# broadinstitute/gatk-bwamem-jni

Hardware: AMD Instinct MI355X
Metric: 150bp reads aligned/sec vs GRCh38-scale reference (1/2/4/8 MI355X) (higher is better)
Workload: dtype u8/int32/int64; 1 GPU; 10000000 x 150bp single-end synthetic reads per GPU vs synthetic GRCh38-scale genome (3100000000 bp, 24 contigs, 5% diverged repeats), full index in HBM; reads_per_gpu=10000000, read_len=150, genome_bp=3100000000, genome=iid, response_bytes=542940344, parallelism=read-sharded x1, no collectives, hip_hw_queues=4, paired_end=False

## Files before the change

gatk-bwamem-jni_amd/csrc/bwamem_types.h:

```cpp
#pragma once
#include <stdint.h>
#include <stddef.h>
#include <hip/hip_runtime.h>

struct MemOpt {
    int a, b;
    int o_del, e_del;
    int o_ins, e_ins;
    int pen_unpaired;
    int pen_clip5, pen_clip3;
    int w;
    int zdrop;
    uint64_t max_mem_intv;
    int T;
    int flag;
    int min_seed_len;
    int min_chain_weight;
    int max_chain_extend;
    float split_factor;
    int split_width;
    int max_occ;
    int max_chain_gap;
    int n_threads;
    int chunk_size;
    float mask_level;
    float drop_ratio;
    float XA_drop_ratio;
    float mask_level_redun;
    float mapQ_coef_len;
    int mapQ_coef_fac;
    int max_ins;
    int max_matesw;
    int max_XA_hits, max_XA_hits_alt;
    int8_t mat[25];
};
static_assert(sizeof(MemOpt) == 168, "mem_opt_t ABI (BwaMemAligner.java:137)");

struct MemPestat { int low, high; int failed; double avg, std; };
static_assert(sizeof(MemPestat) == 32, "mem_pestat_t ABI");

struct PairTab { const double* t; int64_t lo[4]; int32_t n[4], off[4]; };

enum {
    MEM_F_PE = 0x2, MEM_F_NOPAIRING = 0x4, MEM_F_ALL = 0x8, MEM_F_NO_MULTI = 0x10,
    MEM_F_NO_RESCUE = 0x20, MEM_F_PRIMARY5 = 0x800
};

struct DevIndex {
    const uint4* occ;
    const uint32_t* sa_lo;
    const uint8_t*  sa_hi;
    const uint8_t*  pac;
    const int64_t*  ann_offset;
    const int32_t*  ann_len;
    const int32_t*  ann_is_alt;
    const int32_t*  ann_name_off;
    const char*     names;
    const double*   log_tab;
    uint64_t primary, L2[5], seq_len;
    int64_t  l_pac;
    int32_t  n_seqs, sa_intv, log_tab_n, sa_shift;
    int32_t  n_cu, lds_bytes;
};

struct Intv { uint64_t x0, x1, size, info; };

struct Seed { int64_t rbeg; int32_t qbeg, len, score, next; };

struct Chain {
    int64_t pos;
    int32_t n, first, rid;
    uint32_t w;
    int32_t kept, is_alt;
    int32_t seed0;
    int32_t last;
    float frac_rep;
    int32_t pad_;
};

struct AlnReg {
    int64_t rb, re;
    int32_t qb, qe;
    int32_t rid;
    int32_t score, truesc, sub, alt_sc, csub, sub_n, w, seedcov, secondary, secondary_all, seedlen0;
    int32_t n_comp, is_alt;
    float frac_rep;
    int32_t pad_;
    uint64_t hash;
};

struct SwJob { int64_t rb; int32_t read, tag, l_ms, is_rev, tlen, xtra, q_off, pad_; };
struct KswR { int score, te, qe, score2, te2, tb, qb; };

struct DevCounters {
    unsigned long long n_ext, n_lf, n_sa, n_dp_cells, n_ref_bases, n_reads;
    unsigned long long dbg[10];
};

enum { ERR_INTV_CAP = 1, ERR_OUT_CAP = 2, ERR_CIGAR_CAP = 4, ERR_LONG_READ = 8, ERR_SCRATCH = 16, ERR_BTREE = 32, ERR_BAD_REG = 64, ERR_JOB_CAP = 128, ERR_ZPOOL = 256, ERR_RESCUE_CAP = 512 };

#define BT_NODE_INTS 40

struct TileView {
    int32_t n_reads;
    int32_t max_len;
    int64_t read_id0;
    const int64_t* seq_off;
    uint8_t* seq;
    int32_t intv_cap;
    Intv* intv;
    int32_t* n_intv;
    Intv* smem_scratch;
    int32_t smem_cap;
    int32_t* l_rep;
    int32_t* n_seeds;
// ... 32 lines not shown
```

gatk-bwamem-jni_amd/csrc/k_seed.hip:

```cpp
#include "dev_common.h"
#include "wave_ops.h"
#include "kernels.h"

DEV uint32_t mask16(int n)
{
    n = n < 0 ? 0 : n > 16 ? 16 : n;
    return (uint32_t)(0x5555555500000000ull >> (n << 1));
}
DEV void cnt_word_m(uint32_t x, uint32_t m, uint32_t& c1, uint32_t& c2, uint32_t& c3)
{
    const uint32_t lo = x & m, hi = (x >> 1) & m;
    c3 += __popc(hi & lo);
    c2 += __popc(hi & ~lo);
    c1 += __popc(~hi & lo);
}
DEV void extend_sm(const DevIndex& ix, uint64_t x0, uint64_t x1, uint64_t size, int c, bool is_back, uint64_t& o0, uint64_t& o1, uint64_t& osz)
{
    const uint64_t xa = is_back ? x0 : x1, xb = is_back ? x1 : x0;
    const uint64_t k = xa - 1, l = xa - 1 + size;
    const uint64_t kk = k - (k >= ix.primary), ll = l - (l >= ix.primary);
    const uint64_t bk = kk >> 6, bl = ll >> 6;
    const uint4* pk = ix.occ + 2 * bk;
    const uint4* pl = ix.occ + 2 * bl;
    const uint4 ck = pk[0], sk = pk[1], cl = pl[0], sl = pl[1];
    const int nk = (int)(kk & 63) + 1, nl = (int)(ll & 63) + 1;
    uint32_t a1 = 0, a2 = 0, a3 = 0, b1 = 0, b2 = 0, b3 = 0;
    cnt_word_m(sk.x, mask16(nk), a1, a2, a3);       cnt_word_m(sl.x, mask16(nl), b1, b2, b3);
    cnt_word_m(sk.y, mask16(nk - 16), a1, a2, a3);  cnt_word_m(sl.y, mask16(nl - 16), b1, b2, b3);
    cnt_word_m(sk.z, mask16(nk - 32), a1, a2, a3);  cnt_word_m(sl.z, mask16(nl - 32), b1, b2, b3);
    cnt_word_m(sk.w, mask16(nk - 48), a1, a2, a3);  cnt_word_m(sl.w, mask16(nl - 48), b1, b2, b3);
    const uint64_t tk1 = ((uint64_t)(ck.w & 0xffu) << 32 | ck.x) + a1, tk2 = ((uint64_t)(ck.w >> 8 & 0xffu) << 32 | ck.y) + a2, tk3 = ((uint64_t)(ck.w >> 16 & 0xffu) << 32 | ck.z) + a3;
    const uint64_t tl1 = ((uint64_t)(cl.w & 0xffu) << 32 | cl.x) + b1, tl2 = ((uint64_t)(cl.w >> 8 & 0xffu) << 32 | cl.y) + b2, tl3 = ((uint64_t)(cl.w >> 16 & 0xffu) << 32 | cl.z) + b3;
    const uint64_t s1 = tl1 - tk1, s2 = tl2 - tk2, s3 = tl3 - tk3;
    const uint64_t s0 = (ll - kk) - s1 - s2 - s3;
    const uint64_t tk0 = kk + 1 - tk1 - tk2 - tk3;
    const uint64_t tkc = c == 0 ? tk0 : c == 1 ? tk1 : c == 2 ? tk2 : tk3;
    const uint64_t sc = c == 0 ? s0 : c == 1 ? s1 : c == 2 ? s2 : s3;
    const uint64_t l2c = c == 0 ? ix.L2[0] : c == 1 ? ix.L2[1] : c == 2 ? ix.L2[2] : ix.L2[3];
    uint64_t other = xb + (xa <= ix.primary && xa + size - 1 >= ix.primary);
    other += (c < 3 ? s3 : 0) + (c < 2 ? s2 : 0) + (c < 1 ? s1 : 0);
    const uint64_t na = l2c + 1 + tkc;
    o0 = is_back ? na : other;
    o1 = is_back ? other : na;
    osz = sc;
}

struct CandStack {
    uint32_t *v0, *v1, *v2;
    uint16_t* v2n;
    uint4* spill;
    int K, spill_cap;
    bool narrow;
    static __device__ uint32_t pack2(uint64_t x0, uint64_t size, int end) { return (uint32_t)(x0 >> 32) | (uint32_t)(size >> 32) << 5 | (uint32_t)end << 10; }
    __device__ uint32_t hi_get(int e) const {
        const int s = (e & (K - 1)) * 64;
        if (!narrow) return v2[s];
        const uint32_t h = v2n[s];
        return (h & 7u) | (h >> 3 & 7u) << 5 | (h >> 6) << 10;
    }
    __device__ void hi_put(int e, uint32_t w2) {
        const int s = (e & (K - 1)) * 64;
        if (!narrow) v2[s] = w2;
        else v2n[s] = (uint16_t)((w2 & 7u) | (w2 >> 5 & 7u) << 3 | (w2 >> 10) << 6);
    }
    __device__ bool push(int e, uint64_t x0, uint64_t size, int end) {
        const int s = (e & (K - 1)) * 64;
        if (e >= K) {
            if (e - K >= spill_cap) return false;
            uint4 t; t.x = v0[s]; t.y = v1[s]; t.z = hi_get(e); t.w = 0;
            spill[(size_t)(e - K) * 64] = t;
        }
        v0[s] = (uint32_t)x0; v1[s] = (uint32_t)size; hi_put(e, pack2(x0, size, end));
        return true;
    }
    __device__ void put(int e, int n, uint64_t x0, uint64_t size, int end) {
        if (e >= n - K) { const int s = (e & (K - 1)) * 64; v0[s] = (uint32_t)x0; v1[s] = (uint32_t)size; hi_put(e, pack2(x0, size, end)); }
        else { uint4 t; t.x = (uint32_t)x0; t.y = (uint32_t)size; t.z = pack2(x0, size, end); t.w = 0; spill[(size_t)e * 64] = t; }
    }
    __device__ void get(int e, int n, uint64_t& x0, uint64_t& size, int& end) const {
        uint32_t a, b, w2;
        if (e >= n - K) { const int s = (e & (K - 1)) * 64; a = v0[s]; b = v1[s]; w2 = hi_get(e); }
        else { const uint4 t = spill[(size_t)e * 64]; a = t.x; b = t.y; w2 = t.z; }
        x0 = (uint64_t)(w2 & 31) << 32 | a; size = (uint64_t)(w2 >> 5 & 31) << 32 | b; end = (int)(w2 >> 10);
    }
};

__global__ void k_encode(uint8_t* seq, int64_t n_bytes)
{
    int64_t i = (int64_t)blockIdx.x * blockDim.x + threadIdx.x;
    int64_t stride = (int64_t)gridDim.x * blockDim.x;
    for (; i < n_bytes; i += stride) {
        uint8_t c = seq[i];
        if (c >= 4) {
            uint8_t u = c & 0xdf;
            c = u == 'A' ? 0 : u == 'C' ? 1 : u == 'G' ? 2 : u == 'T' ? 3 : 4;
            seq[i] = c;
        }
    }
}

enum { S_IDLE = 0, S_NEXT = 1, S_FWD = 2, S_BWD = 3, S_P3 = 4 };
#define SEED_EL_CAP 4

template <bool LDSQ>
__global__ void __launch_bounds__(64) k_seed(DevIndex ix, MemOpt opt, TileView tv, int K, int refill_min, int narrow)
{
    HIP_DYNAMIC_SHARED(uint32_t, lds)
    const int lane = threadIdx.x;
    CandStack V;
    V.narrow = narrow != 0;
    V.v0 = lds + lane; V.v1 = V.v0 + K * 64; V.v2 = V.v1 + K * 64; V.K = K;
    V.v2n = (uint16_t*)(lds + 2 * K * 64) + lane;
    V.spill = (uint4*)tv.smem_scratch + (size_t)blockIdx.x * tv.smem_cap * 64 + lane; V.spill_cap = tv.smem_cap;
    uint32_t* el = lds + (narrow ? 5 * K * 32 : 3 * K * 64) + lane;
    uint32_t* sq = el + SEED_EL_CAP * 64;
    unsigned int* work = (unsigned int*)(tv.err + 8);
    const int min_seed_len = opt.min_seed_len;
    const int split_len = (int)(opt.min_seed_len * opt.split_factor + .499);
    const uint64_t max_intv3 = (uint64_t)(int64_t)(int)opt.max_mem_intv;

    int st = S_IDLE, r = 0, len = 0, pass = 1, x = 0, sx = 0, i = 0, k2 = 0, old_n = 0, mem_n = 0;
    int nf = 0, lo = 0, rd = 0, wr = 0, c = -1, ret = 0, end = 0, n_el = 0;
    uint64_t min_intv = 1, last_start = 0, last_sz = 0, ik0 = 0, ik1 = 0, iks = 0;
    bool any = false, ovf = false, exhausted = false, el_ok = true;
    const uint8_t* qg = tv.seq;
    Intv* mem = tv.intv;
    uint32_t n_ext = 0;

    uint64_t qwin = 0;
    const uint8_t* qwin_at = nullptr;
    auto qat_g = [&](int p) -> int {
        const uint8_t* a = qg + p;
        const uint8_t* al = a - ((uintptr_t)a & 7);
        if (al != qwin_at) { qwin_at = al; qwin = *(const uint64_t*)al; }
        return (int)(qwin >> (((uintptr_t)a & 7) << 3) & 0xffu);
    };
#define QAT(p) (LDSQ ? (int)(sq[((p) >> 3) * 64] >> (((p) & 7) << 2) & 15u) : qat_g(p))
#define FINISH() do { fin = true; st = S_IDLE; } while (0)
#define MEM_PUSH(X0, SZ, INFO) do { if (mem_n >= tv.intv_cap) ovf = true; else { Intv v_; v_.x0 = (X0); v_.x1 = 0; v_.size = (SZ); v_.info = (INFO); mem[mem_n++] = v_; } } while (0)
#define PUSH_IK() do { if (V.push(nf, ik0, iks, end)) ++nf; else ovf = true; } while (0)
#define BEGIN_BWD() do { ret = end; lo = 0; rd = wr = nf - 1; i = sx - 1; c = i >= 0 ? QAT(i) : 4; c = c < 4 ? c : -1; st = S_BWD; } while (0)

    for (;;) {
        bool fin = false;
        const unsigned long long idle = __ballot(st == S_IDLE);
        if (idle != 0ull && !exhausted && (__popcll(idle) >= refill_min || idle == ~0ull)) {
            const int n_need = __popcll(idle);
            unsigned int base = 0;
            if (lane == 0) base = atomicAdd(work, (unsigned int)n_need);
            base = (unsigned int)__shfl((int)base, 0);
            if (base + (unsigned int)n_need >= (unsigned int)tv.n_reads) exhausted = true;
            bool fresh = false;
            if (st == S_IDLE) {
                const unsigned int cand = base + (unsigned int)__popcll(idle & ((1ull << lane) - 1ull));
                if (cand < (unsigned int)tv.n_reads) {
                    r = (int)cand; fresh = true;
                    const int64_t off = tv.seq_off[r];
                    len = (int)(tv.seq_off[r + 1] - off - 1);
                    qg = tv.seq + off;
                    mem = tv.intv + (size_t)r * tv.intv_cap;
                    mem_n = 0; ovf = false; pass = 1; x = 0; st = S_NEXT; n_el = 0; el_ok = true;
                }
            }
            if (LDSQ) {
                unsigned long long got = __ballot(fresh);
                while (got) {
                    const int l = __ffsll((long long)got) - 1;
                    got &= got - 1ull;
                    const int rr = __shfl(r, l);
                    const int64_t off = tv.seq_off[rr];
                    const int nb = (int)(tv.seq_off[rr + 1] - off) - 1;
                    for (int k = lane; k * 8 < nb; k += 64) {
                        uint32_t wd = 0;
                        uint32_t by[8];
#pragma unroll
                        for (int b = 0; b < 8; ++b) { const int pos = k * 8 + b; by[b] = tv.seq[off + (pos < nb ? pos : nb)]; }
#pragma unroll
                        for (int b = 0; b < 8; ++b) wd |= (k * 8 + b < nb ? by[b] & 15u : 4u) << (b << 2);
                        sq[k * 64 + (l - lane)] = wd;
                    }
                }
                __syncthreads();
            }
            if (fresh && len < min_seed_len) { tv.n_intv[r] = 0; st = S_IDLE; }
        }
        if (__ballot(st != S_IDLE) == 0ull) break;

        if (st == S_NEXT) {
            int nx = -1;
            bool p3 = false;
            uint64_t nmin = 1;
            if (pass == 1) {
                if (x >= len) { pass = 2; old_n = mem_n; k2 = 0; }
                else if (QAT(x) > 3) ++x;
                else nx = x;
            } else if (pass == 2 && el_ok) {
                if (k2 >= n_el) { pass = 3; x = 0; if (!(opt.max_mem_intv > 0)) FINISH(); }
                else {
                    const uint32_t wd = el[k2 * 64];
                    const int m = (int)(wd & 0x1ffffu);
                    if (QAT(m) > 3) ++k2;
                    else { nx = m; nmin = (uint64_t)(wd >> 17) + 1; }
                }
            } else if (pass == 2) {
                if (k2 >= old_n) { pass = 3; x = 0; if (!(opt.max_mem_intv > 0)) FINISH(); }
                else {
                    const uint64_t psz = mem[k2].size, pinfo = mem[k2].info;
                    const int s0 = (int)(pinfo >> 32), e0 = (int)(int32_t)pinfo;
                    if (e0 - s0 < split_len || psz > (uint64_t)(int64_t)opt.split_width) ++k2;
                    else {
                        const int m = (s0 + e0) >> 1;
                        if (QAT(m) > 3) ++k2;
                        else { nx = m; nmin = psz + 1; }
                    }
                }
            } else {
                if (x >= len) FINISH();
                else if (QAT(x) > 3) ++x;
                else { nx = x; p3 = true; }
            }
            if (nx >= 0) {
                const int b = QAT(nx);
                const uint64_t lb = b == 0 ? ix.L2[0] : b == 1 ? ix.L2[1] : b == 2 ? ix.L2[2] : ix.L2[3];
                const uint64_t lb1 = b == 0 ? ix.L2[1] : b == 1 ? ix.L2[2] : b == 2 ? ix.L2[3] : ix.L2[4];
                const uint64_t lc = b == 0 ? ix.L2[3] : b == 1 ? ix.L2[2] : b == 2 ? ix.L2[1] : ix.L2[0];
                ik0 = lb + 1; iks = lb1 - lb; ik1 = lc + 1;
                sx = nx; i = sx + 1;
                if (p3) st = S_P3;
                else { min_intv = nmin; end = sx + 1; nf = 0; any = false; st = S_FWD; }
            }
        }

        bool need = false, bw = false, back = false;
        int rc = 0, pend = 0;
        uint64_t r0 = 0, r1 = 0, rs = 0;
        bool fwd_end = false;
        if (st == S_FWD || st == S_P3) {
            const int cq = i < len ? QAT(i) : 4;
            if (cq < 4) { need = true; rc = 3 - cq; r0 = ik0; r1 = ik1; rs = iks; }
            else if (st == S_FWD) fwd_end = true;
            else { x = i < len ? i + 1 : len; st = S_NEXT; }
        }
        if (st == S_BWD) {
            V.get(rd, nf, r0, rs, pend);
            bw = true;
            if (c >= 0) { need = true; back = true; rc = c; }
        }

        uint64_t o0 = 0, o1 = 0, os = 0, em0 = 0, ems = 0, emi = 0;
        bool emit = false;
        if (need) { extend_sm(ix, r0, r1, rs, rc, back, o0, o1, os); ++n_ext; }

        if (bw) {
            if (!need || os < min_intv) {
                if (wr == nf - 1 && (!any || (uint64_t)(i + 1) < last_start)) {
                    any = true; last_start = (uint64_t)(i + 1);
                    if (pend - (i + 1) >= min_seed_len) {
                        emit = true; em0 = r0; ems = rs; emi = (uint64_t)(i + 1) << 32 | (uint32_t)pend;
                        if (pass == 1 && pend - (i + 1) >= split_len && rs <= (uint64_t)(int64_t)opt.split_width) {
                            if (n_el < SEED_EL_CAP && rs < 32768u) el[n_el * 64] = (uint32_t)((i + 1 + pend) >> 1) | (uint32_t)rs << 17;
                            else el_ok = false;
                            ++n_el;
                        }
                    }
                }
            } else if (wr == nf - 1 || os != last_sz) {
                V.put(wr, nf, o0, os, pend); --wr; last_sz = os;
            }
            --rd;
            if (rd < lo) {
                if (wr == nf - 1) { if (pass == 1) x = ret; else ++k2; st = S_NEXT; }
                else { lo = wr + 1; rd = wr = nf - 1; --i; c = i >= 0 ? QAT(i) : 4; c = c < 4 ? c : -1; }
            }
        } else if (st == S_FWD && (need || fwd_end)) {
            const bool push = fwd_end || os != iks;
            const bool stop = fwd_end || (push && os < min_intv);
            if (push) PUSH_IK();
            if (stop) BEGIN_BWD();
            else { ik0 = o0; ik1 = o1; iks = os; end = i + 1; ++i; }
        } else if (need) {
            if (os < max_intv3 && i - sx >= min_seed_len) {
                if (os > 0) { emit = true; em0 = o0; ems = os; emi = (uint64_t)sx << 32 | (uint32_t)(i + 1); }
                x = i + 1; st = S_NEXT;
            } else { ik0 = o0; ik1 = o1; iks = os; ++i; }
        }
        if (emit) MEM_PUSH(em0, ems, emi);
        if (ovf) FINISH();
        if (fin) {
            tv.n_intv[r] = ovf ? 0 : mem_n;
            if (ovf) atomicOr(tv.err, ERR_INTV_CAP);
        }
    }
#undef QAT
#undef FINISH
#undef MEM_PUSH
#undef PUSH_IK
#undef BEGIN_BWD
    unsigned long long tot = n_ext;
    for (int o = 32; o > 0; o >>= 1) tot += __shfl_down(tot, o);
    if (lane == 0) { count_add(&tv.cnt->n_ext, tot); }
}

__global__ void k_seed_fin(MemOpt opt, TileView tv)
{
    const int r = blockIdx.x * blockDim.x + threadIdx.x;
    if (r >= tv.n_reads) return;
    Intv* a = tv.intv + (size_t)r * tv.intv_cap;
    const int n = tv.n_intv[r];
    for (int i = 1; i < n; ++i) {
        Intv t = a[i];
        int j = i;
        while (j > 0 && a[j - 1].info > t.info) { a[j] = a[j - 1]; --j; }
        a[j] = t;
    }
    int n_seeds = 0, l_rep = 0, b = 0, e = 0;
    int32_t* iso = tv.intv_seed_off + (size_t)r * tv.intv_cap;
    for (int i = 0; i < n; ++i) {
        const Intv p = a[i];
        const int sb = (int)(p.info >> 32), se = (int)(uint32_t)p.info;
        iso[i] = n_seeds;
        {
            int64_t step = p.size > (uint64_t)(int64_t)opt.max_occ ? (int64_t)(p.size / (uint64_t)opt.max_occ) : 1;
            int64_t c = ((int64_t)p.size + step - 1) / step;
            n_seeds += (int)(c < opt.max_occ ? c : opt.max_occ);
        }
        if (p.size <= (uint64_t)(int64_t)opt.max_occ) continue;
        if (sb > e) { l_rep += e - b; b = sb; e = se; }
        else e = e > se ? e : se;
    }
    l_rep += e - b;
    tv.n_seeds[r] = n_seeds;
    tv.l_rep[r] = l_rep;
}

__global__ void __launch_bounds__(1024) k_scan(const int32_t* in, int64_t* out, int n)
{
    __shared__ int64_t wtot[2][16];
    const int t = threadIdx.x, lane = t & 63, wv = t >> 6;
    int64_t carry = 0;
    int ph = 0;
    for (int base = 0; base < n; base += 4096, ph ^= 1) {
        const int i0 = base + t * 4;
        int v0 = 0, v1 = 0, v2 = 0, v3 = 0;
        if (i0 + 3 < n) { const int4 q = *(const int4*)(in + i0); v0 = q.x; v1 = q.y; v2 = q.z; v3 = q.w; }
        else { if (i0 < n) v0 = in[i0]; if (i0 + 1 < n) v1 = in[i0 + 1]; if (i0 + 2 < n) v2 = in[i0 + 2]; }
        const int64_t sum = (int64_t)v0 + v1 + v2 + v3;
        int64_t incl = sum;
        for (int o = 1; o < 64; o <<= 1) { int64_t u = __shfl_up(incl, o); if (lane >= o) incl += u; }
        if (lane == 63) wtot[ph][wv] = incl;
        __syncthreads();
        int64_t pre = carry, tot = 0;
        for (int w = 0; w < 16; ++w) { const int64_t x = wtot[ph][w]; if (w < wv) pre += x; tot += x; }
        int64_t run = pre + incl - sum;
// ... 177 lines not shown
    if (ix.sa_intv == src_intv) return;
    if (t == 0) v = ix.seq_len;
    const uint64_t smask = (uint64_t)src_intv - 1, dmask = (uint64_t)ix.sa_intv - 1;
    for (uint64_t step = 0; ; ++step) {
        if (step > ix.seq_len) { atomicOr(err, ERR_SCRATCH); return; }
        k = lf_step(ix, k);
        if (!(k & smask)) return;
        --v;
        if (!(k & dmask)) { lo[k >> ix.sa_shift] = (uint32_t)v; hi[k >> ix.sa_shift] = (uint8_t)(v >> 32); }
    }
}

void launch_sa_densify(hipStream_t st, const DevIndex& ix, const uint64_t* sa_src, uint64_t n_src, int src_intv, uint32_t* lo, uint8_t* hi, int32_t* err)
{
    hipLaunchKernelGGL(k_sa_densify, dim3((unsigned)((n_src + 255) / 256)), dim3(256), 0, st, ix, sa_src, n_src, src_intv, lo, hi, err);
}

__global__ void k_build_occ64(const uint32_t* bwt, uint64_t n_blocks, uint4* occ)
{
    uint64_t b = (uint64_t)blockIdx.x * blockDim.x + threadIdx.x;
    if (b >= n_blocks) return;
    const uint32_t* blk = bwt + (b >> 1 << 4);
    const uint64_t* cnt = (const uint64_t*)blk;
    const uint32_t* sym = blk + 8 + ((b & 1) << 2);
    uint32_t c1 = 0, c2 = 0, c3 = 0;
    if (b & 1) for (int i = 0; i < 4; ++i) cnt_word(blk[8 + i], 16, c1, c2, c3);
    const uint64_t C = cnt[1] + c1, G = cnt[2] + c2, T = cnt[3] + c3;
    uint4 c, s;
    c.x = (uint32_t)C; c.y = (uint32_t)G; c.z = (uint32_t)T;
    c.w = (uint32_t)(C >> 32 & 0xff) | (uint32_t)(G >> 32 & 0xff) << 8 | (uint32_t)(T >> 32 & 0xff) << 16;
    s.x = sym[0]; s.y = sym[1]; s.z = sym[2]; s.w = sym[3];
    occ[2 * b] = c; occ[2 * b + 1] = s;
}

void launch_build_occ64(hipStream_t st, const uint32_t* bwt, uint64_t n_blocks, uint4* occ)
{
    hipLaunchKernelGGL(k_build_occ64, dim3((unsigned)((n_blocks + 255) / 256)), dim3(256), 0, st, bwt, n_blocks, occ);
}

__global__ void k_unpack_pac(const uint8_t* pac, int64_t start, int64_t n, uint8_t* dst)
{
    int64_t i = (int64_t)blockIdx.x * blockDim.x + threadIdx.x;
    const int64_t stride = (int64_t)gridDim.x * blockDim.x;
    for (; i < n; i += stride) dst[i] = (uint8_t)pac_base(pac, start + i);
}
void launch_unpack_pac(hipStream_t st, const DevIndex& ix, int64_t start, int64_t n, uint8_t* dst)
{
    if (n <= 0) return;
    int64_t nb = (n + 255) / 256;
    if (nb > 65536) nb = 65536;
    hipLaunchKernelGGL(k_unpack_pac, dim3((unsigned)nb), dim3(256), 0, st, ix.pac, start, n, dst);
}

void launch_encode(hipStream_t st, uint8_t* seq, int64_t n_bytes)
{
    if (n_bytes <= 0) return;
    int64_t nb = (n_bytes + 255) / 256;
    if (nb > 8192) nb = 8192;
    hipLaunchKernelGGL(k_encode, dim3((unsigned)nb), dim3(256), 0, st, seq, n_bytes);
}
void launch_seed(hipStream_t st, const DevIndex& ix, const MemOpt& opt, const TileView& tv)
{
    if (tv.n_reads <= 0) return;
    const int n_cu = ix.n_cu > 0 ? ix.n_cu : 256;
    int K = 16, wpc = 0, refill_min = 4;
    { const char* e = getenv("BWAMEM_HIP_SEED_REFILL"); if (e && atoi(e) > 0) refill_min = atoi(e); }
    { const char* e = getenv("BWAMEM_HIP_SEED_K"); if (e && atoi(e) > 0) K = atoi(e); }
    { const char* e = getenv("BWAMEM_HIP_SEED_WPC"); if (e && atoi(e) > 0) wpc = atoi(e); }
    while (K & (K - 1)) K &= K - 1;
    const size_t qbytes = (size_t)64 * 4 * (((size_t)tv.max_len + 7) / 8);
    const bool ldsq = qbytes <= 24576;
    int narrow = ix.seq_len < (1ull << 35) && tv.max_len < 1023;
    { const char* e = getenv("BWAMEM_HIP_SEED_NARROW"); if (e) narrow = narrow && atoi(e) != 0; }
    const size_t lds = (size_t)(narrow ? 5 * K * 32 : 3 * K * 64) * 4 + (size_t)SEED_EL_CAP * 64 * 4 + (ldsq ? qbytes : 0) + 16;
    if (!wpc) { wpc = (int)((size_t)(160 * 1024) / ((lds + 1023) & ~(size_t)1023)); wpc = wpc < 1 ? 1 : wpc > 16 ? 16 : wpc; }
    const int groups = (tv.n_reads + 63) / 64;
    int grid = groups < n_cu * wpc ? groups : n_cu * wpc;
    if (tv.smem_groups > 0 && grid > tv.smem_groups) grid = tv.smem_groups;
    if (ldsq) hipLaunchKernelGGL(k_seed<true>, dim3(grid), dim3(64), lds, st, ix, opt, tv, K, refill_min, narrow);
    else hipLaunchKernelGGL(k_seed<false>, dim3(grid), dim3(64), lds, st, ix, opt, tv, K, refill_min, narrow);
    hipLaunchKernelGGL(k_seed_fin, dim3((tv.n_reads + 255) / 256), dim3(256), 0, st, opt, tv);
}
size_t scan_tmp_bytes(int64_t n) { return (size_t)((n + 4095) / 4096 + 2) * 8; }
static int scan_knob(const char* name, int dflt) { const char* e = getenv(name); return e && atoi(e) > 0 ? atoi(e) : dflt; }
void launch_scan(hipStream_t st, const int32_t* in, int64_t* out, int n, int64_t* tmp)
{
    const int single_max = scan_knob("BWAMEM_HIP_SCAN_SINGLE_MAX", 8192), fused_max = scan_knob("BWAMEM_HIP_SCAN_FUSED_MAX", 2048);
    if (n <= single_max || !tmp) { hipLaunchKernelGGL(k_scan, dim3(1), dim3(1024), 0, st, in, out, n); return; }
    const int nb = (n + 4095) / 4096;
    hipLaunchKernelGGL(k_scan_part, dim3(nb), dim3(256), 0, st, in, n, tmp);
    if (nb <= fused_max) { hipLaunchKernelGGL(k_scan_apply<true>, dim3(nb), dim3(256), 0, st, in, n, (const int64_t*)tmp, out); return; }
    hipLaunchKernelGGL(k_scan_top, dim3(1), dim3(64), 0, st, tmp, nb, out + n);
    hipLaunchKernelGGL(k_scan_apply<false>, dim3(nb), dim3(256), 0, st, in, n, (const int64_t*)tmp, out);
}
size_t nul_tmp_bytes(int64_t n_bytes) { const size_t nb = (size_t)((n_bytes + 15) / 4096 + 2); return nb * 4 + 128 + (nb + 1) * 8 + scan_tmp_bytes((int64_t)nb); }
void launch_nul_offsets(hipStream_t st, const uint8_t* seq, int64_t n_bytes, int64_t* off, int64_t n_reads_max, int64_t* n_found, void* tmp)
{
    const int nb = (int)((n_bytes + 4095) / 4096);
    int32_t* cnt = (int32_t*)tmp;
    int64_t* blk_off = (int64_t*)((char*)tmp + (((size_t)(nb + 2) * 4 + 63) & ~(size_t)63));
    int64_t* scan_tmp = blk_off + nb + 1;
    (void)hipMemsetAsync(off, 0, 8, st);
    if (nb <= 0) { (void)hipMemsetAsync(n_found, 0, 8, st); return; }
    hipLaunchKernelGGL(k_nul_count, dim3(nb), dim3(256), 0, st, seq, n_bytes, cnt);
    launch_scan(st, cnt, blk_off, nb, scan_tmp);
    hipLaunchKernelGGL(k_nul_write, dim3(nb), dim3(256), 0, st, seq, n_bytes, (const int64_t*)blk_off, nb, off, n_reads_max, n_found);
}
void launch_sa(hipStream_t st, const DevIndex& ix, const MemOpt& opt, const TileView& tv, int64_t n_occ)
{
    if (n_occ <= 0) return;
    hipLaunchKernelGGL(k_sa, dim3((unsigned)((n_occ + 255) / 256)), dim3(256), 0, st, ix, opt, tv, n_occ);
}
```

gatk-bwamem-jni_amd/csrc/kernels.h:

```cpp
#pragma once
#include <hip/hip_runtime.h>
#include "bwamem_types.h"
#include "bam_encode.h"

void launch_build_occ64(hipStream_t st, const uint32_t* bwt, uint64_t n_blocks, uint4* occ);
void launch_sa_densify(hipStream_t st, const DevIndex& ix, const uint64_t* sa_src, uint64_t n_src, int src_intv, uint32_t* lo, uint8_t* hi, int32_t* err);
void launch_encode(hipStream_t st, uint8_t* seq, int64_t n_bytes);
void launch_unpack_pac(hipStream_t st, const DevIndex& ix, int64_t start, int64_t n, uint8_t* dst);
void launch_seed(hipStream_t st, const DevIndex& ix, const MemOpt& opt, const TileView& tv);
size_t scan_tmp_bytes(int64_t n);
void launch_scan(hipStream_t st, const int32_t* in, int64_t* out, int n, int64_t* tmp);
void launch_order(hipStream_t st, const int32_t* n_seeds, int n, int32_t* bins64, int32_t* order);
size_t nul_tmp_bytes(int64_t n_bytes);
void launch_nul_offsets(hipStream_t st, const uint8_t* seq, int64_t n_bytes, int64_t* off, int64_t n_reads_max, int64_t* n_found, void* tmp);
void launch_sa(hipStream_t st, const DevIndex& ix, const MemOpt& opt, const TileView& tv, int64_t n_occ);
void launch_chain(hipStream_t st, const DevIndex& ix, const MemOpt& opt, const TileView& tv, Chain* chain_store);
bool rescore_needed(const MemOpt& opt, const TileView& tv);
void launch_rescore(hipStream_t st, const DevIndex& ix, const MemOpt& opt, const TileView& tv, void* jobs, void* results, int32_t* first_num, int32_t* cnt, int cap);
size_t extend_lds_bytes(const MemOpt& opt, int max_len);
void launch_extend(hipStream_t st, const DevIndex& ix, const MemOpt& opt, const TileView& tv);
void launch_post1(hipStream_t st, const DevIndex& ix, const MemOpt& opt, const TileView& tv);
void launch_final_prep(hipStream_t st, const DevIndex& ix, const MemOpt& opt, const TileView& tv);
size_t gcigar_slab_bytes(const MemOpt& opt, int max_len);
int gcigar_slab_grid(const DevIndex& ix, int n_jobs);
void launch_gcigar(hipStream_t st, const DevIndex& ix, const MemOpt& opt, const TileView& tv, int n_jobs, const void* jobs, void* outs, uint32_t* cig_pool, int cig_cap,
                   uint8_t* zpool, unsigned long long zpool_cap, unsigned long long* zpool_cur, uint8_t* slabs, size_t slab_bytes, int* queue);
void launch_final_se(hipStream_t st, const DevIndex& ix, const MemOpt& opt, const TileView& tv, const void* job_out, const uint32_t* job_cig, int cig_cap);
void launch_pack(hipStream_t st, const TileView& tv, uint8_t* dst);
void launch_bam_size(hipStream_t st, const BamTile& t);
void launch_bam_emit(hipStream_t st, const BamTile& t);

void launch_pestat_cand(hipStream_t st, const DevIndex& ix, const MemOpt& opt, const TileView& tv, int8_t* cand_dir, int64_t* cand_is);
void launch_pe_caps(hipStream_t st, const MemOpt& opt, const TileView& tv, int32_t* caps);
void launch_pe_copy_regs(hipStream_t st, const TileView& tv, const AlnReg* src, const int64_t* src_off, AlnReg* dst, const int64_t* dst_off, const int32_t* n_regs);
void launch_pe_pair(hipStream_t st, const DevIndex& ix, const MemOpt& opt, const TileView& tv, AlnReg* regs, const int64_t* reg_off,
                    int32_t* n_regs, int32_t* ints, void* vpool, void* keys, uint8_t* scratch, int64_t scratch_per_pair, int cap_h, int cap_b, int cap_u, const MemPestat* pes, const PairTab& ptab, void* states,
                    void* rescue_jobs, void* rescue_res, int32_t* rescue_first, int32_t* rescue_num, int32_t* rescue_cnt, int rescue_cap);
size_t pe_rescue_bytes(int what, int cap);
void launch_sw_jobs(hipStream_t st, const DevIndex& ix, const MemOpt& opt, const TileView& tv, const void* jobs, const int32_t* cnt, int cap, void* results, int cap_b, int max_qlen);
void launch_pe_out(hipStream_t st, const DevIndex& ix, const MemOpt& opt, const TileView& tv, AlnReg* regs, const int64_t* reg_off,
                   int32_t* n_regs, int32_t* ints, const MemPestat* pes, const void* states, const void* job_out, const uint32_t* job_cig, int cig_cap);
size_t pe_state_bytes(int n_reads);
```

gatk-bwamem-jni_amd/csrc/pipeline.cpp:

```cpp
#include <hip/hip_runtime.h>
#include <stdio.h>
#include <stdlib.h>
#include <string.h>
#include <math.h>
#include <unistd.h>
#include <fcntl.h>
#include <errno.h>
#include <time.h>
#include <sys/stat.h>
#include <sys/mman.h>
#include <dlfcn.h>
#include <mutex>
#include <condition_variable>
#include <thread>
#include <atomic>
#include <functional>
#include <memory>
#include <string>
#include <vector>
#include <deque>
#include <stdexcept>
#include <algorithm>
#include <cmath>
#include "bwamem_types.h"
// ... 138 lines not shown
    }
};

struct ReqBuf {
    DevBuf seq, off, tmp;
    int64_t* h_off = nullptr; size_t h_cap = 0;
    ~ReqBuf() { if (h_off) (void)hipHostFree(h_off); }
    bool ensure_host(size_t n) {
        if (n <= h_cap) return true;
        if (h_off) (void)hipHostFree(h_off);
        h_off = nullptr; h_cap = 0;
        n += n / 8 + 64;
        if (hipHostMalloc((void**)&h_off, n * 8, hipHostMallocDefault) != hipSuccess) { h_off = nullptr; return false; }
        h_cap = n;
        return true;
    }
};

struct CapHints {
    std::mutex mu;
    double jobs_per_read = 0, zpool_mult = 1;
    double seeds_per_read = 0;
    int out_cap = 512;
    void saw_seeds(int T, int64_t n_occ) { std::lock_guard<std::mutex> lk(mu); if (T >= 1024) seeds_per_read = seeds_per_read == 0 ? (double)n_occ / T : 0.75 * seeds_per_read + 0.25 * (double)n_occ / T; }
    int tile_scale() { std::lock_guard<std::mutex> lk(mu); return seeds_per_read > 32 ? 2 : 1; }
    void learn(int T, int n_jobs, double zpool_mult_, int out_cap_) {
        std::lock_guard<std::mutex> lk(mu);
        if (T >= 64) jobs_per_read = std::max(jobs_per_read, 1.25 * n_jobs / T);
        zpool_mult = std::min(64.0, std::max(zpool_mult, zpool_mult_));
        out_cap = std::max(out_cap, out_cap_);
    }
    void get(int T, int& jobs, double& zpool_mult_, int& out_cap_) {
        std::lock_guard<std::mutex> lk(mu);
        jobs = (int)std::min(1.0e9, jobs_per_read * T) + 1; zpool_mult_ = zpool_mult; out_cap_ = out_cap;
    }
    double pe_rescue_per_read = 0, pe_jobs_per_read = 0;
    int pe_cap_u = 256;
    void learn_pe(int T, int n_rescue, int n_jobs, int cap_u) {
        std::lock_guard<std::mutex> lk(mu);
        if (T >= 64) { pe_rescue_per_read = std::max(pe_rescue_per_read, 1.25 * n_rescue / T); pe_jobs_per_read = std::max(pe_jobs_per_read, 1.25 * n_jobs / T); }
        pe_cap_u = std::min(2048, std::max(pe_cap_u, cap_u));
    }
    void get_pe(int T, int& rescue, int& jobs, int& cap_u) {
        std::lock_guard<std::mutex> lk(mu);
        rescue = (int)std::min(1.0e9, pe_rescue_per_read * T) + 1; jobs = (int)std::min(1.0e9, pe_jobs_per_read * T) + 1; cap_u = pe_cap_u;
    }
};

struct bwaidx_s {
    uint8_t* mem = nullptr; size_t l_mem = 0; bool mmapped = false;
    HostIndex h;
    int device = 0;
    DevIndex d;
    DevBuf d_occ, d_sa_lo, d_sa_hi, d_pac, d_ann_off, d_ann_len, d_ann_alt, d_name_off, d_names, d_log, d_ptab;
    PairTab pair_tab;
    std::mutex mu;
    Workspace ws;
    std::vector<std::unique_ptr<Workspace>> extra_ws;
    Workspace seed_ws;
    SeedStore seed_store[SEED_STORES_MAX];
    CapHints hints;
    std::vector<std::unique_ptr<ReqBuf>> req_bufs;
    hipStream_t up_stream = nullptr;
    std::vector<bwaidx_s*> peers;
    std::atomic<uint32_t> next_replica{0};
    std::mutex split_mu;
    ~bwaidx_s() { if (up_stream) (void)hipStreamDestroy(up_stream); }
};

struct TileOut {
    uint8_t* d = nullptr; size_t bytes = 0; bool owned = false;
    int64_t* d_off = nullptr; int64_t read_id = 0; int n_reads = 0, max_len = 0;
};

struct PeTile { uint32_t r0 = 0; int T = 0, L = 0; uint8_t* seq = nullptr; const int64_t* seq_off = nullptr; DevBuf n_regs, regs, reg_off; int64_t n_regs_total = 0; std::vector<int8_t> cand_dir; std::vector<int64_t> cand_is; };
struct PeCall { std::deque<PeTile> tiles; int64_t read_id0 = 0; };

struct OutSink {
    bool to_host = false;
    std::mutex mu; std::condition_variable cv;
    std::deque<int64_t> bytes, start;
    size_t n_placed = 0; int64_t placed_end = 0;
    uint64_t reads_total = 0, reads_known = 0;
    uint8_t* h_buf = nullptr; size_t h_cap = 0; int inflight = 0;
    DevBuf pool; size_t last_total = 0;
    bool aborted = false;
    void begin_call(uint64_t n_reads) {
        std::lock_guard<std::mutex> lk(mu);
        bytes.clear(); start.clear(); n_placed = 0; placed_end = 0; reads_total = n_reads; reads_known = 0; inflight = 0; aborted = false;
        if (h_buf) { free(h_buf); h_buf = nullptr; } h_cap = 0;
    }
    void add_tiles(size_t n) { std::lock_guard<std::mutex> lk(mu); bytes.resize(bytes.size() + n, -1); start.resize(start.size() + n, 0); }
    void abort() { { std::lock_guard<std::mutex> lk(mu); aborted = true; } cv.notify_all(); }
    bool place(size_t i, int64_t nbytes, int n_reads, uint8_t** dst) {
        std::unique_lock<std::mutex> lk(mu);
        bytes[i] = nbytes; reads_known += (uint64_t)n_reads;
        cv.notify_all();
        cv.wait(lk, [&] {
            while (n_placed < bytes.size() && bytes[n_placed] >= 0) { start[n_placed] = placed_end; placed_end += bytes[n_placed]; ++n_placed; }
            return aborted || n_placed > i;
        });
        if (aborted) return false;
        const size_t need = (size_t)(start[i] + nbytes);
        if (!to_host) { *dst = pool.p && need <= pool.bytes ? pool.as<uint8_t>() + start[i] : nullptr; return true; }
        if (need > h_cap) {
            cv.wait(lk, [&] { return aborted || inflight == 0; });
            if (aborted) return false;
// ... 64 lines not shown
    if (!ix->d_pac.ensure((size_t)(h.l_pac / 4 + 1) + 16)) return false;
    HIP_OK(hipMemcpy(ix->d_pac.p, h.pac, (size_t)(h.l_pac / 4 + 1), hipMemcpyHostToDevice));
    std::vector<int64_t> off(n); std::vector<int32_t> len(n), alt(n), noff(n + 1);
    std::string names;
    for (int i = 0; i < n; ++i) {
        off[i] = h.contigs[i].offset; len[i] = h.contigs[i].len; alt[i] = h.contigs[i].is_alt;
        noff[i] = (int32_t)names.size();
        names += h.contigs[i].name; names.push_back('\0');
    }
    noff[n] = (int32_t)names.size();
    if (!ix->d_ann_off.ensure((size_t)n * 8 + 8) || !ix->d_ann_len.ensure((size_t)n * 4 + 4) || !ix->d_ann_alt.ensure((size_t)n * 4 + 4)
        || !ix->d_name_off.ensure((size_t)(n + 1) * 4) || !ix->d_names.ensure(names.size() + 1) || !ix->d_log.ensure((size_t)LOG_TAB_N * 8)) return false;
    HIP_OK(hipMemcpy(ix->d_ann_off.p, off.data(), (size_t)n * 8, hipMemcpyHostToDevice));
    HIP_OK(hipMemcpy(ix->d_ann_len.p, len.data(), (size_t)n * 4, hipMemcpyHostToDevice));
    HIP_OK(hipMemcpy(ix->d_ann_alt.p, alt.data(), (size_t)n * 4, hipMemcpyHostToDevice));
    HIP_OK(hipMemcpy(ix->d_name_off.p, noff.data(), (size_t)(n + 1) * 4, hipMemcpyHostToDevice));
    HIP_OK(hipMemcpy(ix->d_names.p, names.data(), names.size(), hipMemcpyHostToDevice));
    {
        std::vector<double> lt(LOG_TAB_N);
        for (int i = 0; i < LOG_TAB_N; ++i) lt[i] = log((double)i);
        HIP_OK(hipMemcpy(ix->d_log.p, lt.data(), (size_t)LOG_TAB_N * 8, hipMemcpyHostToDevice));
    }
    DevIndex& d = ix->d;
    memset(&d, 0, sizeof d);
    d.occ = ix->d_occ.as<uint4>(); d.pac = ix->d_pac.as<uint8_t>();
    d.ann_offset = ix->d_ann_off.as<int64_t>(); d.ann_len = ix->d_ann_len.as<int32_t>(); d.ann_is_alt = ix->d_ann_alt.as<int32_t>();
    d.ann_name_off = ix->d_name_off.as<int32_t>(); d.names = ix->d_names.as<char>(); d.log_tab = ix->d_log.as<double>();
    d.primary = h.primary; for (int i = 0; i < 5; ++i) d.L2[i] = h.L2[i];
    d.seq_len = h.seq_len; d.l_pac = h.l_pac; d.n_seqs = n; d.log_tab_n = LOG_TAB_N;
    {
        int v = 0;
        d.n_cu = hipDeviceGetAttribute(&v, hipDeviceAttributeMultiprocessorCount, ix->device) == hipSuccess && v > 0 ? v : 256;
        d.lds_bytes = hipDeviceGetAttribute(&v, hipDeviceAttributeMaxSharedMemoryPerBlock, ix->device) == hipSuccess && v > 0 ? v : 64 << 10;
    }
    {
        int dense = 1;
        if (const char* e = getenv("BWAMEM_HIP_SA_INTV")) { dense = atoi(e); if (dense < 1 || (dense & (dense - 1))) dense = 1; }
        size_t free_b = 0, total_b = 0;
        HIP_OK(hipMemGetInfo(&free_b, &total_b));
        if (dense > h.sa_intv) dense = h.sa_intv;
        while (dense < h.sa_intv && ((size_t)(h.seq_len / dense) + 1) * 5 + (size_t)h.n_sa * 8 > free_b / 4) dense <<= 1;
        d.sa_intv = dense; d.sa_shift = 0;
        while ((1 << d.sa_shift) < dense) ++d.sa_shift;
        const size_t n_kept = (size_t)(h.seq_len >> d.sa_shift) + 1;
        DevBuf src, flag;
        if (!ix->d_sa_lo.ensure(n_kept * 4 + 64) || !ix->d_sa_hi.ensure(n_kept + 64) || !src.ensure((size_t)h.n_sa * 8) || !flag.ensure(64)) return false;
        d.sa_lo = ix->d_sa_lo.as<uint32_t>(); d.sa_hi = ix->d_sa_hi.as<uint8_t>();
        int32_t bad = 1;
        if (hipMemcpy(src.p, h.sa, (size_t)h.n_sa * 8, hipMemcpyHostToDevice) == hipSuccess && hipMemset(flag.p, 0, 64) == hipSuccess) {
            launch_sa_densify(0, d, src.as<uint64_t>(), h.n_sa, h.sa_intv, ix->d_sa_lo.as<uint32_t>(), ix->d_sa_hi.as<uint8_t>(), flag.as<int32_t>());
            if (hipDeviceSynchronize() != hipSuccess || hipMemcpy(&bad, flag.p, 4, hipMemcpyDeviceToHost) != hipSuccess) bad = 1;
        }
        if (bad) { fprintf(stderr, "[bwamem_hip] suffix array densification failed\n"); return false; }
    }
    return true;
}

struct Roctx {
    int (*push)(const char*) = nullptr; int (*pop)() = nullptr;
    Roctx() {
        if (const char* e = getenv("BWAMEM_HIP_ROCTX")) if (atoi(e) == 0) return;
        for (const char* lib : { "librocprofiler-sdk-roctx.so", "librocprofiler-sdk-roctx.so.1", "libroctx64.so", "libroctx64.so.4" }) {
            void* h = dlopen(lib, RTLD_LAZY | RTLD_LOCAL);
            if (!h) continue;
            push = (int (*)(const char*))dlsym(h, "roctxRangePushA"); pop = (int (*)())dlsym(h, "roctxRangePop");
            if (push && pop) return;
            push = nullptr; pop = nullptr;
        }
    }
};
static Roctx& roctx() { static Roctx r; return r; }
struct RoctxRange { bool on; RoctxRange(const char* name) : on(roctx().push != nullptr) { if (on) roctx().push(name); } ~RoctxRange() { if (on) roctx().pop(); } };

static void timed_begin(Workspace& ws, KernelId id)
{
    if (!g_stats.enabled) return;
    Timed t; t.id = id;
    if (hipEventCreate(&t.a) != hipSuccess || hipEventCreate(&t.b) != hipSuccess) return;
    (void)hipEventRecord(t.a, ws.stream);
    ws.timed.push_back(t);
}
static void timed_end(Workspace& ws)
{
    if (!g_stats.enabled || ws.timed.empty()) return;
    (void)hipEventRecord(ws.timed.back().b, ws.stream);
}
static void timed_collect(Workspace& ws)
{
    if (ws.timed.empty()) return;
    std::lock_guard<std::mutex> lk(g_stats.mu);
    for (Timed& t : ws.timed) {
        float ms = 0;
        if (hipEventElapsedTime(&ms, t.a, t.b) == hipSuccess) {
            double* slot[K_N] = { &g_stats.s.ms_encode, &g_stats.s.ms_seed, &g_stats.s.ms_sa, &g_stats.s.ms_chain, &g_stats.s.ms_extend,
                                  &g_stats.s.ms_post, &g_stats.s.ms_final, &g_stats.s.ms_pack, &g_stats.s.ms_other };
            *slot[t.id] += ms;
            if (t.id == K_SEED) ++g_stats.s.n_launch_seed;
            if (t.id == K_SA) ++g_stats.s.n_launch_sa;
            if (t.id == K_EXTEND) ++g_stats.s.n_launch_extend;
        }
        (void)hipEventDestroy(t.a); (void)hipEventDestroy(t.b);
    }
    ws.timed.clear();
}
static int g_verbose = -1;
static bool verbose() { if (g_verbose < 0) { const char* e = getenv("BWAMEM_HIP_VERBOSE"); g_verbose = e && atoi(e) > 0; } return g_verbose > 0; }
// ... 1368 lines not shown
```

Baseline: 23.43 million reads/s.

## Add k-mer lookup table for seeding pass 3 and split it into own kernel

Builds a device-resident table of FM-index SA intervals for all k-mers (k up to 14, chosen from genome size and free memory) at index load. Pass-3 seeding then starts each forward extension from the table entry instead of doing k backward-search steps from a single base. Pass 3 also moves out of the wave-cooperative k_seed kernel into a separate thread-per-read kernel, k_seed_p3, which is on by default. This trades extra HBM for the table, a one-time build and an extra launch for fewer occ lookups. It also risks load imbalance in the simple per-thread kernel.

```diff
diff --git a/gatk-bwamem-jni_amd/csrc/bwamem_types.h b/gatk-bwamem-jni_amd/csrc/bwamem_types.h
--- a/gatk-bwamem-jni_amd/csrc/bwamem_types.h
+++ b/gatk-bwamem-jni_amd/csrc/bwamem_types.h
@@ -61,6 +61,8 @@
     int64_t  l_pac;
     int32_t  n_seqs, sa_intv, log_tab_n, sa_shift;
     int32_t  n_cu, lds_bytes;
+    const uint4* kmer_tab;
+    int32_t  kmer_k, pad_;
 };
 
 struct Intv { uint64_t x0, x1, size, info; };
diff --git a/gatk-bwamem-jni_amd/csrc/k_seed.hip b/gatk-bwamem-jni_amd/csrc/k_seed.hip
--- a/gatk-bwamem-jni_amd/csrc/k_seed.hip
+++ b/gatk-bwamem-jni_amd/csrc/k_seed.hip
@@ -45,6 +45,39 @@
     osz = sc;
 }
 
+DEV uint4 kmer_pack(uint64_t x0, uint64_t x1, uint64_t size)
+{
+    uint4 e;
+    e.x = (uint32_t)x0; e.y = (uint32_t)x1; e.z = (uint32_t)size;
+    e.w = (uint32_t)(x0 >> 32 & 0xff) | (uint32_t)(x1 >> 32 & 0xff) << 8 | (uint32_t)(size >> 32 & 0xff) << 16;
+    return e;
+}
+DEV void kmer_unpack(const uint4 e, uint64_t& x0, uint64_t& x1, uint64_t& size)
+{
+    x0 = (uint64_t)(e.w & 0xffu) << 32 | e.x; x1 = (uint64_t)(e.w >> 8 & 0xffu) << 32 | e.y; size = (uint64_t)(e.w >> 16 & 0xffu) << 32 | e.z;
+}
+DEV void base_intv(const DevIndex& ix, int b, uint64_t& x0, uint64_t& x1, uint64_t& size)
+{
+    const uint64_t lb = b == 0 ? ix.L2[0] : b == 1 ? ix.L2[1] : b == 2 ? ix.L2[2] : ix.L2[3];
+    const uint64_t lb1 = b == 0 ? ix.L2[1] : b == 1 ? ix.L2[2] : b == 2 ? ix.L2[3] : ix.L2[4];
+    const uint64_t lc = b == 0 ? ix.L2[3] : b == 1 ? ix.L2[2] : b == 2 ? ix.L2[1] : ix.L2[0];
+    x0 = lb + 1; size = lb1 - lb; x1 = lc + 1;
+}
+__global__ void __launch_bounds__(256) k_kmer_level(DevIndex ix, const uint4* parent, uint4* child, uint32_t n_parent)
+{
+    const uint32_t t = blockIdx.x * blockDim.x + threadIdx.x;
+    if (t >= n_parent) return;
+    uint4 e[4];
+    uint64_t p0 = 0, p1 = 0, ps = 0, x0, x1, sz;
+    if (parent) kmer_unpack(parent[t], p0, p1, ps);
+    for (int b = 0; b < 4; ++b) {
+        if (parent) extend_sm(ix, p0, p1, ps, 3 - b, false, x0, x1, sz);
+        else base_intv(ix, b, x0, x1, sz);
+        e[b] = kmer_pack(x0, x1, sz);
+    }
+    for (int b = 0; b < 4; ++b) child[4 * (size_t)t + b] = e[b];
+}
+
 struct CandStack {
     uint32_t *v0, *v1, *v2;
     uint16_t* v2n;
@@ -102,7 +135,7 @@
 enum { S_IDLE = 0, S_NEXT = 1, S_FWD = 2, S_BWD = 3, S_P3 = 4 };
 #define SEED_EL_CAP 4
 
-template <bool LDSQ>
+template <bool LDSQ, bool P3 = true>
 __global__ void __launch_bounds__(64) k_seed(DevIndex ix, MemOpt opt, TileView tv, int K, int refill_min, int narrow)
 {
     HIP_DYNAMIC_SHARED(uint32_t, lds)
@@ -195,7 +228,7 @@
                 else if (QAT(x) > 3) ++x;
                 else nx = x;
             } else if (pass == 2 && el_ok) {
-                if (k2 >= n_el) { pass = 3; x = 0; if (!(opt.max_mem_intv > 0)) FINISH(); }
+                if (k2 >= n_el) { pass = 3; x = 0; if (!P3 || !(opt.max_mem_intv > 0)) FINISH(); }
                 else {
                     const uint32_t wd = el[k2 * 64];
                     const int m = (int)(wd & 0x1ffffu);
@@ -203,7 +236,7 @@
                     else { nx = m; nmin = (uint64_t)(wd >> 17) + 1; }
                 }
             } else if (pass == 2) {
-                if (k2 >= old_n) { pass = 3; x = 0; if (!(opt.max_mem_intv > 0)) FINISH(); }
+                if (k2 >= old_n) { pass = 3; x = 0; if (!P3 || !(opt.max_mem_intv > 0)) FINISH(); }
                 else {
                     const uint64_t psz = mem[k2].size, pinfo = mem[k2].info;
                     const int s0 = (int)(pinfo >> 32), e0 = (int)(int32_t)pinfo;
@@ -220,13 +253,16 @@
                 else { nx = x; p3 = true; }
             }
             if (nx >= 0) {
-                const int b = QAT(nx);
-                const uint64_t lb = b == 0 ? ix.L2[0] : b == 1 ? ix.L2[1] : b == 2 ? ix.L2[2] : ix.L2[3];
-                const uint64_t lb1 = b == 0 ? ix.L2[1] : b == 1 ? ix.L2[2] : b == 2 ? ix.L2[3] : ix.L2[4];
-                const uint64_t lc = b == 0 ? ix.L2[3] : b == 1 ? ix.L2[2] : b == 2 ? ix.L2[1] : ix.L2[0];
-                ik0 = lb + 1; iks = lb1 - lb; ik1 = lc + 1;
+                base_intv(ix, QAT(nx), ik0, ik1, iks);
                 sx = nx; i = sx + 1;
-                if (p3) st = S_P3;
+                if (p3) {
+                    st = S_P3;
+                    if (ix.kmer_tab && ix.kmer_k <= min_seed_len && nx + ix.kmer_k <= len) {
+                        uint32_t km = 0; bool acgt = true;
+                        for (int j = 0; j < ix.kmer_k; ++j) { const int b = QAT(nx + j); acgt = acgt && b < 4; km = km << 2 | (uint32_t)(b & 3); }
+                        if (acgt) { kmer_unpack(ix.kmer_tab[km], ik0, ik1, iks); i = sx + ix.kmer_k; }
+                    }
+                }
                 else { min_intv = nmin; end = sx + 1; nf = 0; any = false; st = S_FWD; }
             }
         }
@@ -287,7 +323,7 @@
         if (emit) MEM_PUSH(em0, ems, emi);
         if (ovf) FINISH();
         if (fin) {
-            tv.n_intv[r] = ovf ? 0 : mem_n;
+            tv.n_intv[r] = ovf ? (P3 ? 0 : -1) : mem_n;
             if (ovf) atomicOr(tv.err, ERR_INTV_CAP);
         }
     }
@@ -299,6 +335,66 @@
     unsigned long long tot = n_ext;
     for (int o = 32; o > 0; o >>= 1) tot += __shfl_down(tot, o);
     if (lane == 0) { count_add(&tv.cnt->n_ext, tot); }
+}
+
+__global__ void __launch_bounds__(256) k_seed_p3(DevIndex ix, MemOpt opt, TileView tv)
+{
+    const int r = blockIdx.x * blockDim.x + threadIdx.x;
+    const int min_seed_len = opt.min_seed_len;
+    const uint64_t max_intv3 = (uint64_t)(int64_t)(int)opt.max_mem_intv;
+    uint32_t n_ext = 0;
+    if (r < tv.n_reads) {
+        const int n0 = tv.n_intv[r];
+        const int64_t off = tv.seq_off[r];
+        const int len = (int)(tv.seq_off[r + 1] - off - 1);
+        if (n0 < 0) tv.n_intv[r] = 0;
+        else if (len >= min_seed_len && opt.max_mem_intv > 0) {
+            const uint8_t* qg = tv.seq + off;
+            uint64_t qwin = 0;
+            const uint8_t* qwin_at = nullptr;
+            auto qat = [&](int p) -> int {
+                const uint8_t* a = qg + p;
+                const uint8_t* al = a - ((uintptr_t)a & 7);
+                if (al != qwin_at) { qwin_at = al; qwin = *(const uint64_t*)al; }
+                return (int)(qwin >> (((uintptr_t)a & 7) << 3) & 0xffu);
+            };
+            const bool tab = ix.kmer_tab && ix.kmer_k <= min_seed_len;
+            Intv* mem = tv.intv + (size_t)r * tv.intv_cap;
+            int mem_n = n0, x = 0, sx = 0, i = 0;
+            uint64_t ik0 = 0, ik1 = 0, iks = 0;
+            bool fresh = true, ovf = false;
+            for (;;) {
+                if (fresh) {
+                    while (x < len && qat(x) > 3) ++x;
+                    if (x >= len) break;
+                    base_intv(ix, qat(x), ik0, ik1, iks);
+                    sx = x; i = x + 1; fresh = false;
+                    if (tab && x + ix.kmer_k <= len) {
+                        uint32_t km = 0; bool acgt = true;
+                        for (int j = 0; j < ix.kmer_k; ++j) { const int b = qat(x + j); acgt = acgt && b < 4; km = km << 2 | (uint32_t)(b & 3); }
+                        if (acgt) { kmer_unpack(ix.kmer_tab[km], ik0, ik1, iks); i = x + ix.kmer_k; }
+                    }
+                }
+                const int cq = i < len ? qat(i) : 4;
+                if (cq > 3) { x = i < len ? i + 1 : len; fresh = true; continue; }
+                uint64_t o0, o1, os;
+                extend_sm(ix, ik0, ik1, iks, 3 - cq, false, o0, o1, os); ++n_ext;
+                if (os < max_intv3 && i - sx >= min_seed_len) {
+                    if (os > 0) {
+                        if (mem_n >= tv.intv_cap) { ovf = true; break; }
+                        Intv v; v.x0 = o0; v.x1 = 0; v.size = os; v.info = (uint64_t)sx << 32 | (uint32_t)(i + 1);
+                        mem[mem_n++] = v;
+                    }
+                    x = i + 1; fresh = true;
+                } else { ik0 = o0; ik1 = o1; iks = os; ++i; }
+            }
+            if (ovf) { tv.n_intv[r] = 0; atomicOr(tv.err, ERR_INTV_CAP); }
+            else if (mem_n != n0) tv.n_intv[r] = mem_n;
+        }
+    }
+    unsigned long long tot = n_ext;
+    for (int o = 32; o > 0; o >>= 1) tot += __shfl_down(tot, o);
+    if ((threadIdx.x & 63) == 0 && tot) count_add(&tv.cnt->n_ext, tot);
 }
 
 __global__ void k_seed_fin(MemOpt opt, TileView tv)
@@ -582,6 +678,23 @@
     hipLaunchKernelGGL(k_unpack_pac, dim3((unsigned)nb), dim3(256), 0, st, ix.pac, start, n, dst);
 }
 
+int kmer_tab_k(uint64_t seq_len)
+{
+    int k = 0;
+    while (k < 14 && (1ull << (2 * (k + 1))) <= seq_len / 4) ++k;
+    return k >= 2 ? k : 0;
+}
+void launch_kmer_tab(hipStream_t st, const DevIndex& ix, int k, uint4* a, uint4* b)
+{
+    const uint4* parent = nullptr;
+    for (int j = 1; j <= k; ++j) {
+        uint4* child = (k - j) & 1 ? b : a;
+        const uint32_t n = 1u << (2 * (j - 1));
+        hipLaunchKernelGGL(k_kmer_level, dim3((n + 255) / 256), dim3(256), 0, st, ix, parent, child, n);
+        parent = child;
+    }
+}
+
 void launch_encode(hipStream_t st, uint8_t* seq, int64_t n_bytes)
 {
     if (n_bytes <= 0) return;
@@ -607,8 +720,16 @@
     const int groups = (tv.n_reads + 63) / 64;
     int grid = groups < n_cu * wpc ? groups : n_cu * wpc;
     if (tv.smem_groups > 0 && grid > tv.smem_groups) grid = tv.smem_groups;
-    if (ldsq) hipLaunchKernelGGL(k_seed<true>, dim3(grid), dim3(64), lds, st, ix, opt, tv, K, refill_min, narrow);
-    else hipLaunchKernelGGL(k_seed<false>, dim3(grid), dim3(64), lds, st, ix, opt, tv, K, refill_min, narrow);
+    bool split = true;
+    { const char* e = getenv("BWAMEM_HIP_P3_SPLIT"); if (e && atoi(e) == 0) split = false; }
+    if (split) {
+        if (ldsq) hipLaunchKernelGGL((k_seed<true, false>), dim3(grid), dim3(64), lds, st, ix, opt, tv, K, refill_min, narrow);
+        else hipLaunchKernelGGL((k_seed<false, false>), dim3(grid), dim3(64), lds, st, ix, opt, tv, K, refill_min, narrow);
+        hipLaunchKernelGGL(k_seed_p3, dim3((tv.n_reads + 255) / 256), dim3(256), 0, st, ix, opt, tv);
+    } else {
+        if (ldsq) hipLaunchKernelGGL((k_seed<true, true>), dim3(grid), dim3(64), lds, st, ix, opt, tv, K, refill_min, narrow);
+        else hipLaunchKernelGGL((k_seed<false, true>), dim3(grid), dim3(64), lds, st, ix, opt, tv, K, refill_min, narrow);
+    }
     hipLaunchKernelGGL(k_seed_fin, dim3((tv.n_reads + 255) / 256), dim3(256), 0, st, opt, tv);
 }
 size_t scan_tmp_bytes(int64_t n) { return (size_t)((n + 4095) / 4096 + 2) * 8; }
diff --git a/gatk-bwamem-jni_amd/csrc/kernels.h b/gatk-bwamem-jni_amd/csrc/kernels.h
--- a/gatk-bwamem-jni_amd/csrc/kernels.h
+++ b/gatk-bwamem-jni_amd/csrc/kernels.h
@@ -5,6 +5,8 @@
 
 void launch_build_occ64(hipStream_t st, const uint32_t* bwt, uint64_t n_blocks, uint4* occ);
 void launch_sa_densify(hipStream_t st, const DevIndex& ix, const uint64_t* sa_src, uint64_t n_src, int src_intv, uint32_t* lo, uint8_t* hi, int32_t* err);
+int kmer_tab_k(uint64_t seq_len);
+void launch_kmer_tab(hipStream_t st, const DevIndex& ix, int k, uint4* a, uint4* b);
 void launch_encode(hipStream_t st, uint8_t* seq, int64_t n_bytes);
 void launch_unpack_pac(hipStream_t st, const DevIndex& ix, int64_t start, int64_t n, uint8_t* dst);
 void launch_seed(hipStream_t st, const DevIndex& ix, const MemOpt& opt, const TileView& tv);
diff --git a/gatk-bwamem-jni_amd/csrc/pipeline.cpp b/gatk-bwamem-jni_amd/csrc/pipeline.cpp
--- a/gatk-bwamem-jni_amd/csrc/pipeline.cpp
+++ b/gatk-bwamem-jni_amd/csrc/pipeline.cpp
@@ -214,7 +214,7 @@
     HostIndex h;
     int device = 0;
     DevIndex d;
-    DevBuf d_occ, d_sa_lo, d_sa_hi, d_pac, d_ann_off, d_ann_len, d_ann_alt, d_name_off, d_names, d_log, d_ptab;
+    DevBuf d_occ, d_sa_lo, d_sa_hi, d_pac, d_ann_off, d_ann_len, d_ann_alt, d_name_off, d_names, d_log, d_ptab, d_kmer;
     PairTab pair_tab;
     std::mutex mu;
     Workspace ws;
@@ -385,6 +385,25 @@
             if (hipDeviceSynchronize() != hipSuccess || hipMemcpy(&bad, flag.p, 4, hipMemcpyDeviceToHost) != hipSuccess) bad = 1;
         }
         if (bad) { fprintf(stderr, "[bwamem_hip] suffix array densification failed\n"); return false; }
+    }
+    {
+        int k = kmer_tab_k(h.seq_len);
+        if (const char* e = getenv("BWAMEM_HIP_P3_K")) { k = atoi(e); if (k < 2 || k > 14) k = 0; }
+        size_t free_b = 0, total_b = 0;
+        HIP_OK(hipMemGetInfo(&free_b, &total_b));
+        while (k >= 2 && ((size_t)20 << (2 * k)) > free_b / 4) --k;
+        if (k >= 2) {
+            struct timespec t0, t1; clock_gettime(CLOCK_MONOTONIC, &t0);
+            DevBuf scratch;
+            if (!ix->d_kmer.ensure((size_t)16 << (2 * k)) || !scratch.ensure((size_t)4 << (2 * k))) return false;
+            launch_kmer_tab(0, d, k, ix->d_kmer.as<uint4>(), scratch.as<uint4>());
+            if (hipDeviceSynchronize() != hipSuccess) { fprintf(stderr, "[bwamem_hip] k-mer table build failed\n"); return false; }
+            clock_gettime(CLOCK_MONOTONIC, &t1);
+            d.kmer_tab = ix->d_kmer.as<uint4>(); d.kmer_k = k;
+            if (getenv("BWAMEM_HIP_VERBOSE") && atoi(getenv("BWAMEM_HIP_VERBOSE")) > 0)
+                fprintf(stderr, "[bwamem_hip] device %d: %d-mer table of seeding pass 3, %.1f MB, built in %.1f ms\n", ix->device, k,
+                        (double)((size_t)16 << (2 * k)) / 1e6, ((t1.tv_sec - t0.tv_sec) + (t1.tv_nsec - t0.tv_nsec) * 1e-9) * 1e3);
+        }
     }
     return true;
 }
```

Result: no change. 23.20 million reads/s (-1.0%).
